# 18281818221/kalle-audio

Hardware: AMD Instinct MI355X
Metric: audio-seconds/sec (node) DiT train step, 10s@12.5Hz x1024 latents (higher is better)
Workload: dtype bf16; 1 GPU; DiT train step (fwd+bwd+allreduce+Adam), 24 blocks D=1536 h=24, 10 s @ 12.5 Hz x 1024 latents (T=125+1 prepend), S=130 x 768 cross-attn cond; DiT shape chosen by this build (reference defines none); global_batch=256, per_gpu_batch=256, parallelism=dp1, objective=v, io_channels=1024, global_cond_type=prepend

## Files before the change

### kalle_audio_amd/csrc/attention.hip

```cpp
#include "common.h"
#include "../../include/kalle_hip.h"

namespace {

template <int DH>
struct Hd {
    static_assert(DH == 32 || DH == 64 || DH == 128, "head dim 32, 64 or 128");
    static constexpr int STRIDE = 2 * DH + 32;
    static constexpr int TILE = 128 * STRIDE;
    static constexpr float SCALE = DH == 32 ? 0.17677669529663687f : DH == 64 ? 0.125f : 0.08838834764831845f;
    static constexpr float SCALE_LOG2E = SCALE * 1.4426950408889634f;
    static constexpr int PAIRS = DH / 16;
    static constexpr int PAIRS_LOG2 = DH == 32 ? 1 : DH == 64 ? 2 : 3;
    static constexpr int NP = DH == 128 ? 2 : 1;
};
constexpr int AT_STRIDE = Hd<64>::STRIDE;
constexpr int AT_TILE = Hd<64>::TILE;
constexpr float SM_SCALE = Hd<64>::SCALE;
constexpr float NEG_BIG = -1.0e30f;
constexpr float SM_SCALE_LOG2E = Hd<64>::SCALE_LOG2E;
constexpr float LOG2E = 1.4426950408889634f;
constexpr float M_INIT = -2.0e30f;

template <int NT, int DH = 64>
// ... 627 lines not shown
                            dp[t][ot] = __builtin_amdgcn_mfma_f32_16x16x32_bf16(x2, y2[ot][s], dp[t][ot], 0, 0, 0);
                        }
                    }
                    mfma_results_ready();
                    const f32x2 c2 = f32x2{SM_SCALE_LOG2E, SM_SCALE_LOG2E}, sc2 = f32x2{SM_SCALE, SM_SCALE};
                    const int ow = o0 + wave * (16 * OT);
                    const bool diag = p.causal && (KV ? (ow + 16 * OT - 1 > s0 + rb + coff) : (s0 + rb + 15 > ow + coff));
#pragma unroll
                    for (int ot = 0; ot < OT; ++ot) {
                        f32x2 la, lb, da, db;
                        if constexpr (KV) { la = lo2(ra); lb = hi2(ra); da = lo2(rbv); db = hi2(rbv); }
                        else { la = lb = f32x2{ca[ot], ca[ot]}; da = db = f32x2{cb[ot], cb[ot]}; }
                        const f32x2 ea = pk_fma(lo2(sa[t][ot]), c2, la), eb = pk_fma(hi2(sa[t][ot]), c2, lb);
                        f32x4 pv = f32x4{__builtin_amdgcn_exp2f(ea[0]), __builtin_amdgcn_exp2f(ea[1]),
                                         __builtin_amdgcn_exp2f(eb[0]), __builtin_amdgcn_exp2f(eb[1])};
                        if (diag) {
                            const int oi = ow + 16 * ot + li;
#pragma unroll
                            for (int r = 0; r < 4; ++r) {
                                const int si = s0 + rb + 4 * g + r;
                                if (KV ? (oi > si + coff) : (si > oi + coff)) pv[r] = 0.f;
                            }
                        }
                        const f32x2 ta = pk_fma(lo2(dp[t][ot]), sc2, da), tb = pk_fma(hi2(dp[t][ot]), sc2, db);
                        sa[t][ot] = pv;
                        dp[t][ot] = pv * f32x4{ta[0], ta[1], tb[0], tb[1]};
                    }
                }
                bf16x8 pb[OT], dsb[OT];
#pragma unroll
                for (int ot = 0; ot < OT; ++ot) {
                    pb[ot] = pack_pair(sa[0][ot], sa[1][ot]);
                    dsb[ot] = pack_pair(dp[0][ot], dp[1][ot]);
                }
#pragma unroll
                for (int dt = 0; dt < DT; ++dt) {
                    const bf16x8 a1 = trfrag<DH>(R1, 32 * pr, 32 * pr + 16, 16 * dt, lane);
#pragma unroll
                    for (int ot = 0; ot < OT; ++ot)
                        g2[dt][ot] = __builtin_amdgcn_mfma_f32_16x16x32_bf16(a1, dsb[ot], g2[dt][ot], 0, 0, 0);
                    if constexpr (KV) {
                        const bf16x8 a2 = trfrag<DH>(R2, 32 * pr, 32 * pr + 16, 16 * dt, lane);
#pragma unroll
                        for (int ot = 0; ot < OT; ++ot)
                            g1[dt][ot] = __builtin_amdgcn_mfma_f32_16x16x32_bf16(a2, pb[ot], g1[dt][ot], 0, 0, 0);
                    }
                }
            }
        }
    }

    const int nown = KV ? p.Nk : p.Nq;
#pragma unroll
    for (int ot = 0; ot < OT; ++ot) {
        const int oi = o0 + wave * (16 * OT) + 16 * ot + li;
        if (oi >= nown) continue;
        if (p.rot) {
            const int hts = p.rot >> 5;
#pragma unroll
            for (int ht = 0; ht < (DH == 32 ? 1 : 2); ++ht) {
                if (ht >= hts) break;
                const int64_t pos = oi + (KV ? 0 : p.qpos);
                const f32x4 c4 = *reinterpret_cast<const f32x4*>(p.cosT + pos * (p.rot >> 1) + 16 * ht + 4 * g);
                const f32x4 s4 = *reinterpret_cast<const f32x4*>(p.sinT + pos * (p.rot >> 1) + 16 * ht + 4 * g);
                f32x4& lo = hts == 1 ? g2[0][ot] : g2[ht][ot];
                f32x4& hi = hts == 1 ? g2[1][ot] : g2[DH == 32 ? 1 : ht + 2][ot];
#pragma unroll
                for (int r = 0; r < 4; ++r) {
                    const float a = lo[r], bb = hi[r];
                    lo[r] = a * c4[r] + bb * s4[r];
                    hi[r] = bb * c4[r] - a * s4[r];
                }
            }
        }
        if constexpr (KV) {
            bf16_t* dkp = p.dk + ((int64_t)b * p.Nk + oi) * p.ldk + p.k_off + hk * DH + 4 * g;
            bf16_t* dvp = p.dv + ((int64_t)b * p.Nk + oi) * p.ldv + p.v_off + hk * DH + 4 * g;
#pragma unroll
            for (int dt = 0; dt < DT; ++dt) {
                i32x2 w;
                w[0] = (int)pack_bf16x2(g2[dt][ot][0], g2[dt][ot][1]);
                w[1] = (int)pack_bf16x2(g2[dt][ot][2], g2[dt][ot][3]);
                *reinterpret_cast<i32x2*>(dkp + 16 * dt) = w;
                w[0] = (int)pack_bf16x2(g1[dt][ot][0], g1[dt][ot][1]);
                w[1] = (int)pack_bf16x2(g1[dt][ot][2], g1[dt][ot][3]);
                *reinterpret_cast<i32x2*>(dvp + 16 * dt) = w;
            }
        } else {
            bf16_t* dqp = p.dq + ((int64_t)b * p.Nq + oi) * p.ldq + p.q_off + hown * DH + 4 * g;
#pragma unroll
            for (int dt = 0; dt < DT; ++dt) {
                i32x2 w;
                w[0] = (int)pack_bf16x2(g2[dt][ot][0], g2[dt][ot][1]);
                w[1] = (int)pack_bf16x2(g2[dt][ot][2], g2[dt][ot][3]);
                *reinterpret_cast<i32x2*>(dqp + 16 * dt) = w;
            }
        }
    }
}

__device__ __forceinline__ float& row_stat(char* tile, int row, int slot) {
    return *reinterpret_cast<float*>(tile + row * AT_STRIDE + 128 + 4 * slot);
}

__global__ __launch_bounds__(512, 4) __attribute__((amdgpu_waves_per_eu(4, 4))) void attn_bwd_fused_kernel(AttnParams p) {
    constexpr int NT = 512;
    extern __shared__ __attribute__((aligned(16))) char smem[];
    char* RQ = smem;
    char* RD = smem + AT_TILE;
    char* RK = smem + 2 * AT_TILE;
    char* RV = smem + 3 * AT_TILE;
    const int tid = threadIdx.x, lane = tid & 63, wave = tid >> 6;
    const int g = lane >> 4, li = lane & 15;
    const int b = blockIdx.z, h = blockIdx.y;
    const int N = p.Nq, Nk = p.Nk;
    const bf16_t* qb = p.q + (int64_t)b * N * p.ldq + p.q_off + h * 64;
    const bf16_t* kb = p.k + (int64_t)b * Nk * p.ldk + p.k_off + h * 64;
    const bf16_t* vb = p.v + (int64_t)b * Nk * p.ldv + p.v_off + h * 64;
    const bf16_t* dob = p.dout + (int64_t)b * N * p.ldo + h * 64;
    attn_stamp(p, tid, 0);

    {
        TileRegs<NT> tq, td, tk, tv;
        tile_load<NT>(tq, qb, p.ldq, 0, N, p.rot, tid);
        tile_load<NT>(td, dob, p.ldo, 0, N, 0, tid);
        tile_load<NT>(tk, kb, p.ldk, 0, Nk, p.rot, tid);
        tile_load<NT>(tv, vb, p.ldv, 0, Nk, 0, tid);
        const RopeSet<> rq = rope_load(p.cosT, p.sinT, 0, N, p.rot, tid, p.qpos);
        const RopeSet<> rk = rope_load(p.cosT, p.sinT, 0, Nk, p.rot, tid);
        const int drow = tid >> 2, dq4 = tid & 3;
        i32x4 o0v = i32x4{0, 0, 0, 0}, o1v = i32x4{0, 0, 0, 0};
        if (drow < N) {
            const bf16_t* op = p.out + ((int64_t)b * N + drow) * p.ldo + h * 64 + 16 * dq4;
            o0v = *reinterpret_cast<const i32x4*>(op);
            o1v = *reinterpret_cast<const i32x4*>(op + 8);
        }
        float lse_pre = 0.f;
        bool key_ok = drow < Nk;
        if (dq4 == 0 && drow < N) lse_pre = p.lse[((int64_t)b * p.H + h) * N + drow];
        if (dq4 == 1 && key_ok && p.mask) key_ok = p.mask[(int64_t)b * Nk + drow] != 0;
        tile_store<NT>(RQ, tq, 0, N, p.cosT, p.sinT, p.rot, tid, p.qpos, p.rot != 0, rq);
        tile_store<NT>(RD, td, 0, N, nullptr, nullptr, 0, tid);
        tile_store<NT>(RK, tk, 0, Nk, p.cosT, p.sinT, p.rot, tid, 0, p.rot != 0, rk);
        tile_store<NT>(RV, tv, 0, Nk, nullptr, nullptr, 0, tid);
        __syncthreads();
        attn_stamp(p, tid, 1);
        const i32x4 d0v = *reinterpret_cast<const i32x4*>(RD + drow * AT_STRIDE + 32 * dq4);
        const i32x4 d1v = *reinterpret_cast<const i32x4*>(RD + drow * AT_STRIDE + 32 * dq4 + 16);
        float dl = 0.f;
#pragma unroll
        for (int e = 0; e < 4; ++e) {
            dl += bf16lo((uint32_t)o0v[e]) * bf16lo((uint32_t)d0v[e]) + bf16hi((uint32_t)o0v[e]) * bf16hi((uint32_t)d0v[e]);
            dl += bf16lo((uint32_t)o1v[e]) * bf16lo((uint32_t)d1v[e]) + bf16hi((uint32_t)o1v[e]) * bf16hi((uint32_t)d1v[e]);
        }
        dl += __shfl_xor(dl, 1, 64);
        dl += __shfl_xor(dl, 2, 64);
        if (dq4 == 0) {
            const bool ok = drow < N;
            row_stat(RQ, drow, 0) = ok ? -lse_pre * LOG2E : -INFINITY;
            row_stat(RQ, drow, 1) = ok ? -dl * SM_SCALE : 0.f;
            if (ok) p.delta[((int64_t)b * p.H + h) * N + drow] = dl;
        } else if (dq4 == 1) {
            row_stat(RK, drow, 0) = key_ok ? 0.f : -INFINITY;
        }
        __syncthreads();
    }
    attn_stamp(p, tid, 2);
    const f32x2 c2 = f32x2{SM_SCALE_LOG2E, SM_SCALE_LOG2E}, sc2 = f32x2{SM_SCALE, SM_SCALE};
    const int orow = wave * 16;

    if (orow < Nk) {
        bf16x8 y1[2], y2[2];
#pragma unroll
        for (int s = 0; s < 2; ++s) { y1[s] = rowfrag(RK, orow, s, lane); y2[s] = rowfrag(RV, orow, s, lane); }
        const float ca = row_stat(RK, orow + li, 0);
        f32x4 g1[4], g2[4];
#pragma unroll
        for (int dt = 0; dt < 4; ++dt) { g1[dt] = f32x4{0.f, 0.f, 0.f, 0.f}; g2[dt] = f32x4{0.f, 0.f, 0.f, 0.f}; }
#pragma unroll
        for (int pr = 0; pr < 4; ++pr) {
            if (32 * pr >= N) break;
            f32x4 sa[2], dp[2];
#pragma unroll
            for (int t = 0; t < 2; ++t) {
                const int rb = 32 * pr + 16 * t;
                sa[t] = f32x4{ca, ca, ca, ca};
                dp[t] = f32x4{0.f, 0.f, 0.f, 0.f};
#pragma unroll
                for (int s = 0; s < 2; ++s) {
                    sa[t] = __builtin_amdgcn_mfma_f32_16x16x32_bf16(rowfrag(RQ, rb, s, lane), y1[s], sa[t], 0, 0, 0);
                    dp[t] = __builtin_amdgcn_mfma_f32_16x16x32_bf16(rowfrag(RD, rb, s, lane), y2[s], dp[t], 0, 0, 0);
                }
                f32x4 ra, rbv;
#pragma unroll
                for (int r = 0; r < 4; ++r) { ra[r] = row_stat(RQ, rb + 4 * g + r, 0); rbv[r] = row_stat(RQ, rb + 4 * g + r, 1); }
                mfma_results_ready();
                const f32x2 ea = pk_fma(lo2(sa[t]), c2, lo2(ra)), eb = pk_fma(hi2(sa[t]), c2, hi2(ra));
                const f32x4 pv = f32x4{__builtin_amdgcn_exp2f(ea[0]), __builtin_amdgcn_exp2f(ea[1]),
                                       __builtin_amdgcn_exp2f(eb[0]), __builtin_amdgcn_exp2f(eb[1])};
                const f32x2 ta = pk_fma(lo2(dp[t]), sc2, lo2(rbv)), tb = pk_fma(hi2(dp[t]), sc2, hi2(rbv));
                sa[t] = pv;
                dp[t] = pv * f32x4{ta[0], ta[1], tb[0], tb[1]};
            }
            const bf16x8 pb = pack_pair(sa[0], sa[1]), dsb = pack_pair(dp[0], dp[1]);
#pragma unroll
            for (int dt = 0; dt < 4; ++dt) {
                g2[dt] = __builtin_amdgcn_mfma_f32_16x16x32_bf16(trfrag(RQ, 32 * pr, 32 * pr + 16, 16 * dt, lane), dsb, g2[dt], 0, 0, 0);
                g1[dt] = __builtin_amdgcn_mfma_f32_16x16x32_bf16(trfrag(RD, 32 * pr, 32 * pr + 16, 16 * dt, lane), pb, g1[dt], 0, 0, 0);
            }
        }
        attn_stamp(p, tid, 3);
        const int oi = orow + li;
        if (oi < Nk) {
            if (p.rot) {
                const int hts = p.rot >> 5;
#pragma unroll
                for (int ht = 0; ht < 2; ++ht) {
                    if (ht >= hts) break;
                    const f32x4 c4 = *reinterpret_cast<const f32x4*>(p.cosT + (int64_t)oi * (p.rot >> 1) + 16 * ht + 4 * g);
                    const f32x4 s4 = *reinterpret_cast<const f32x4*>(p.sinT + (int64_t)oi * (p.rot >> 1) + 16 * ht + 4 * g);
                    f32x4& lo = hts == 1 ? g2[0] : g2[ht];
                    f32x4& hi = hts == 1 ? g2[1] : g2[ht + 2];
#pragma unroll
                    for (int r = 0; r < 4; ++r) {
                        const float a = lo[r], bb = hi[r];
                        lo[r] = a * c4[r] + bb * s4[r];
                        hi[r] = bb * c4[r] - a * s4[r];
                    }
                }
            }
            store_row64(p.dk + ((int64_t)b * Nk + oi) * p.ldk + p.k_off + h * 64, g2[0], g2[1], g2[2], g2[3], g);
            store_row64(p.dv + ((int64_t)b * Nk + oi) * p.ldv + p.v_off + h * 64, g1[0], g1[1], g1[2], g1[3], g);
        }
    }

    attn_stamp(p, tid, 4);
    if (orow < N) {
        bf16x8 y1[2], y2[2];
#pragma unroll
        for (int s = 0; s < 2; ++s) { y1[s] = rowfrag(RQ, orow, s, lane); y2[s] = rowfrag(RD, orow, s, lane); }
        const float ca = row_stat(RQ, orow + li, 0), cb = row_stat(RQ, orow + li, 1);
        f32x4 g2[4];
#pragma unroll
        for (int dt = 0; dt < 4; ++dt) g2[dt] = f32x4{0.f, 0.f, 0.f, 0.f};
#pragma unroll
        for (int pr = 0; pr < 4; ++pr) {
            if (32 * pr >= Nk) break;
            f32x4 sa[2], dp[2];
#pragma unroll
            for (int t = 0; t < 2; ++t) {
                const int rb = 32 * pr + 16 * t;
#pragma unroll
                for (int r = 0; r < 4; ++r) sa[t][r] = row_stat(RK, rb + 4 * g + r, 0);
                dp[t] = f32x4{0.f, 0.f, 0.f, 0.f};
#pragma unroll
                for (int s = 0; s < 2; ++s) {
                    sa[t] = __builtin_amdgcn_mfma_f32_16x16x32_bf16(rowfrag(RK, rb, s, lane), y1[s], sa[t], 0, 0, 0);
                    dp[t] = __builtin_amdgcn_mfma_f32_16x16x32_bf16(rowfrag(RV, rb, s, lane), y2[s], dp[t], 0, 0, 0);
                }
                mfma_results_ready();
                const f32x2 la = f32x2{ca, ca}, da = f32x2{cb, cb};
                const f32x2 ea = pk_fma(lo2(sa[t]), c2, la), eb = pk_fma(hi2(sa[t]), c2, la);
                const f32x4 pv = f32x4{__builtin_amdgcn_exp2f(ea[0]), __builtin_amdgcn_exp2f(ea[1]),
                                       __builtin_amdgcn_exp2f(eb[0]), __builtin_amdgcn_exp2f(eb[1])};
                const f32x2 ta = pk_fma(lo2(dp[t]), sc2, da), tb = pk_fma(hi2(dp[t]), sc2, da);
                dp[t] = pv * f32x4{ta[0], ta[1], tb[0], tb[1]};
            }
            const bf16x8 dsb = pack_pair(dp[0], dp[1]);
#pragma unroll
            for (int dt = 0; dt < 4; ++dt)
                g2[dt] = __builtin_amdgcn_mfma_f32_16x16x32_bf16(trfrag(RK, 32 * pr, 32 * pr + 16, 16 * dt, lane), dsb, g2[dt], 0, 0, 0);
        }
        const int oi = orow + li;
        if (oi < N) {
            if (p.rot) {
                const int hts = p.rot >> 5;
#pragma unroll
                for (int ht = 0; ht < 2; ++ht) {
                    if (ht >= hts) break;
                    const int64_t pos = oi + p.qpos;
                    const f32x4 c4 = *reinterpret_cast<const f32x4*>(p.cosT + pos * (p.rot >> 1) + 16 * ht + 4 * g);
                    const f32x4 s4 = *reinterpret_cast<const f32x4*>(p.sinT + pos * (p.rot >> 1) + 16 * ht + 4 * g);
                    f32x4& lo = hts == 1 ? g2[0] : g2[ht];
                    f32x4& hi = hts == 1 ? g2[1] : g2[ht + 2];
#pragma unroll
                    for (int r = 0; r < 4; ++r) {
                        const float a = lo[r], bb = hi[r];
                        lo[r] = a * c4[r] + bb * s4[r];
                        hi[r] = bb * c4[r] - a * s4[r];
                    }
                }
            }
            attn_stamp(p, tid, 5);
            store_row64(p.dq + ((int64_t)b * N + oi) * p.ldq + p.q_off + h * 64, g2[0], g2[1], g2[2], g2[3], g);
        }
    }
    if (p.stamps) {
        attn_stamp(p, tid, 6);
        asm volatile("s_waitcnt vmcnt(0)" ::: "memory");
        attn_stamp(p, tid, 7);
    }
}

__global__ __launch_bounds__(512, 4) void attn_bwd_fused_gqa_kernel(AttnParams p) {
    constexpr int NT = 512;
    extern __shared__ __attribute__((aligned(16))) char smem[];
    char* RQ = smem;
    char* RD = smem + AT_TILE;
    char* RK = smem + 2 * AT_TILE;
    char* RV = smem + 3 * AT_TILE;
    const int tid = threadIdx.x, lane = tid & 63, wave = tid >> 6;
    const int g = lane >> 4, li = lane & 15;
    const int b = blockIdx.z, hk = blockIdx.y;
    const int group = p.H / p.Hkv;
    const int N = p.Nq, Nk = p.Nk;
    const int nmain = min(Nk, 128), tail = Nk - nmain;
    const int trow0 = 128 - tail;
    const bf16_t* kb = p.k + (int64_t)b * Nk * p.ldk + p.k_off + hk * 64;
    const bf16_t* vb = p.v + (int64_t)b * Nk * p.ldv + p.v_off + hk * 64;
    const f32x2 c2 = f32x2{SM_SCALE_LOG2E, SM_SCALE_LOG2E}, sc2 = f32x2{SM_SCALE, SM_SCALE};
    const int orow = wave * 16;
    const int drow = tid >> 2, dq4 = tid & 3;

    auto stage_head = [&](int h, bool with_kv, bool write_delta) {
        const bf16_t* qb = p.q + (int64_t)b * N * p.ldq + p.q_off + h * 64;
        const bf16_t* dob = p.dout + (int64_t)b * N * p.ldo + h * 64;
        TileRegs<NT> tq, td, tk, tv;
        tile_load<NT>(tq, qb, p.ldq, 0, N, 0, tid);
        tile_load<NT>(td, dob, p.ldo, 0, N, 0, tid);
        if (with_kv) {
            tile_load<NT>(tk, kb, p.ldk, 0, nmain, 0, tid);
            tile_load<NT>(tv, vb, p.ldv, 0, nmain, 0, tid);
        }
        i32x4 o0v = i32x4{0, 0, 0, 0}, o1v = i32x4{0, 0, 0, 0};
        if (drow < N) {
            const bf16_t* op = p.out + ((int64_t)b * N + drow) * p.ldo + h * 64 + 16 * dq4;
            o0v = *reinterpret_cast<const i32x4*>(op);
            o1v = *reinterpret_cast<const i32x4*>(op + 8);
        }
        i32x4 tkv = i32x4{0, 0, 0, 0}, tvv = i32x4{0, 0, 0, 0};
        const int tj = tid >> 3, tc = tid & 7;
        if (tj < tail) {
            tkv = *reinterpret_cast<const i32x4*>(kb + (int64_t)(128 + tj) * p.ldk + 8 * tc);
            tvv = *reinterpret_cast<const i32x4*>(vb + (int64_t)(128 + tj) * p.ldv + 8 * tc);
        }
        float lse_pre = 0.f;
        bool stat_ok = dq4 == 1 ? drow >= trow0 : drow < nmain;
        if (dq4 == 0 && drow < N) lse_pre = p.lse[((int64_t)b * p.H + h) * N + drow];
        if (dq4 == 1 && stat_ok && p.mask) stat_ok = p.mask[(int64_t)b * Nk + 128 + (drow - trow0)] != 0;
        if (dq4 == 2 && with_kv && stat_ok && p.mask) stat_ok = p.mask[(int64_t)b * Nk + drow] != 0;
        tile_store<NT>(RQ, tq, 0, N, nullptr, nullptr, 0, tid);
        tile_store<NT>(RD, td, 0, N, nullptr, nullptr, 0, tid);
        if (with_kv) {
            tile_store<NT>(RK, tk, 0, nmain, nullptr, nullptr, 0, tid);
            tile_store<NT>(RV, tv, 0, nmain, nullptr, nullptr, 0, tid);
        }
        __syncthreads();
        if (tj < tail) {
            *reinterpret_cast<i32x4*>(RQ + (trow0 + tj) * AT_STRIDE + 16 * tc) = tkv;
            *reinterpret_cast<i32x4*>(RD + (trow0 + tj) * AT_STRIDE + 16 * tc) = tvv;
        }
        const i32x4 d0v = *reinterpret_cast<const i32x4*>(RD + drow * AT_STRIDE + 32 * dq4);
        const i32x4 d1v = *reinterpret_cast<const i32x4*>(RD + drow * AT_STRIDE + 32 * dq4 + 16);
        float dl = 0.f;
#pragma unroll
        for (int e = 0; e < 4; ++e) {
            dl += bf16lo((uint32_t)o0v[e]) * bf16lo((uint32_t)d0v[e]) + bf16hi((uint32_t)o0v[e]) * bf16hi((uint32_t)d0v[e]);
            dl += bf16lo((uint32_t)o1v[e]) * bf16lo((uint32_t)d1v[e]) + bf16hi((uint32_t)o1v[e]) * bf16hi((uint32_t)d1v[e]);
        }
        dl += __shfl_xor(dl, 1, 64);
        dl += __shfl_xor(dl, 2, 64);
        if (dq4 == 0) {
            const bool ok = drow < N;
            row_stat(RQ, drow, 0) = ok ? -lse_pre * LOG2E : -INFINITY;
            row_stat(RQ, drow, 1) = ok ? -dl * SM_SCALE : 0.f;
            if (ok && write_delta) p.delta[((int64_t)b * p.H + h) * N + drow] = dl;
        } else if (dq4 == 1) {
            row_stat(RQ, drow, 2) = stat_ok ? 0.f : -INFINITY;
        } else if (dq4 == 2 && with_kv) {
            row_stat(RK, drow, 0) = stat_ok ? 0.f : -INFINITY;
        }
        __syncthreads();
    };

    auto keys_own = [&](const bf16x8 (&y1)[2], const bf16x8 (&y2)[2], float ca, f32x4 (&gv)[4], f32x4 (&gk)[4]) {
#pragma unroll
        for (int pr = 0; pr < 4; ++pr) {
            if (32 * pr >= N) break;
            f32x4 sa[2], dp[2];
#pragma unroll
            for (int t = 0; t < 2; ++t) {
                const int rb = 32 * pr + 16 * t;
                sa[t] = f32x4{ca, ca, ca, ca};
                dp[t] = f32x4{0.f, 0.f, 0.f, 0.f};
#pragma unroll
                for (int s = 0; s < 2; ++s) {
                    sa[t] = __builtin_amdgcn_mfma_f32_16x16x32_bf16(rowfrag(RQ, rb, s, lane), y1[s], sa[t], 0, 0, 0);
                    dp[t] = __builtin_amdgcn_mfma_f32_16x16x32_bf16(rowfrag(RD, rb, s, lane), y2[s], dp[t], 0, 0, 0);
                }
                f32x4 ra, rbv;
#pragma unroll
                for (int r = 0; r < 4; ++r) { ra[r] = row_stat(RQ, rb + 4 * g + r, 0); rbv[r] = row_stat(RQ, rb + 4 * g + r, 1); }
                mfma_results_ready();
                const f32x2 ea = pk_fma(lo2(sa[t]), c2, lo2(ra)), eb = pk_fma(hi2(sa[t]), c2, hi2(ra));
                f32x4 pv = f32x4{__builtin_amdgcn_exp2f(ea[0]), __builtin_amdgcn_exp2f(ea[1]),
                                 __builtin_amdgcn_exp2f(eb[0]), __builtin_amdgcn_exp2f(eb[1])};
                const f32x2 ta = pk_fma(lo2(dp[t]), sc2, lo2(rbv)), tb = pk_fma(hi2(dp[t]), sc2, hi2(rbv));
                f32x4 ds = pv * f32x4{ta[0], ta[1], tb[0], tb[1]};
#pragma unroll
                for (int r = 0; r < 4; ++r) {
                    if (rb + 4 * g + r >= N) { pv[r] = 0.f; ds[r] = 0.f; }
                }
                sa[t] = pv;
                dp[t] = ds;
            }
            const bf16x8 pb = pack_pair(sa[0], sa[1]), dsb = pack_pair(dp[0], dp[1]);
#pragma unroll
            for (int dt = 0; dt < 4; ++dt) {
                gk[dt] = __builtin_amdgcn_mfma_f32_16x16x32_bf16(trfrag(RQ, 32 * pr, 32 * pr + 16, 16 * dt, lane), dsb, gk[dt], 0, 0, 0);
                gv[dt] = __builtin_amdgcn_mfma_f32_16x16x32_bf16(trfrag(RD, 32 * pr, 32 * pr + 16, 16 * dt, lane), pb, gv[dt], 0, 0, 0);
            }
        }
    };

    {
        stage_head(hk * group, true, true);
        f32x4 g1[4], g2[4];
#pragma unroll
        for (int dt = 0; dt < 4; ++dt) { g1[dt] = f32x4{0.f, 0.f, 0.f, 0.f}; g2[dt] = f32x4{0.f, 0.f, 0.f, 0.f}; }
        for (int hh = 0; hh < group; ++hh) {
            if (hh > 0) {
                __syncthreads();
                stage_head(hk * group + hh, false, true);
            }
            if (orow < nmain) {
                bf16x8 y1[2], y2[2];
#pragma unroll
                for (int s = 0; s < 2; ++s) { y1[s] = rowfrag(RK, orow, s, lane); y2[s] = rowfrag(RV, orow, s, lane); }
                keys_own(y1, y2, row_stat(RK, orow + li, 0), g1, g2);
            }
        }
        const int oi = orow + li;
        if (oi < nmain) {
            store_row64(p.dk + ((int64_t)b * Nk + oi) * p.ldk + p.k_off + hk * 64, g2[0], g2[1], g2[2], g2[3], g);
            store_row64(p.dv + ((int64_t)b * Nk + oi) * p.ldv + p.v_off + hk * 64, g1[0], g1[1], g1[2], g1[3], g);
        }
    }

    for (int hh = group - 1; hh >= 0; --hh) {
        const int h = hk * group + hh;
        if (hh != group - 1) {
            __syncthreads();
            stage_head(h, false, false);
        }
        if (orow < N) {
            bf16x8 y1[2], y2[2];
#pragma unroll
            for (int s = 0; s < 2; ++s) { y1[s] = rowfrag(RQ, orow, s, lane); y2[s] = rowfrag(RD, orow, s, lane); }
            const float ca = row_stat(RQ, orow + li, 0), cb = row_stat(RQ, orow + li, 1);
            f32x4 gq[4];
#pragma unroll
            for (int dt = 0; dt < 4; ++dt) gq[dt] = f32x4{0.f, 0.f, 0.f, 0.f};
            auto stream_keys = [&](const char* SK, const char* SV, int base, auto ext_c) {
                constexpr bool EXT = decltype(ext_c)::value;
                f32x4 dp[2];
#pragma unroll
                for (int t = 0; t < (EXT ? 1 : 2); ++t) {
                    dp[t] = f32x4{0.f, 0.f, 0.f, 0.f};
                    const int rb = base + 16 * t;
                    f32x4 sa;
#pragma unroll
                    for (int r = 0; r < 4; ++r) sa[r] = EXT ? row_stat(RQ, rb + 4 * g + r, 2) : row_stat(RK, rb + 4 * g + r, 0);
#pragma unroll
                    for (int s = 0; s < 2; ++s) {
                        sa = __builtin_amdgcn_mfma_f32_16x16x32_bf16(rowfrag(SK, rb, s, lane), y1[s], sa, 0, 0, 0);
                        dp[t] = __builtin_amdgcn_mfma_f32_16x16x32_bf16(rowfrag(SV, rb, s, lane), y2[s], dp[t], 0, 0, 0);
                    }
                    mfma_results_ready();
                    const f32x2 la = f32x2{ca, ca}, da = f32x2{cb, cb};
                    const f32x2 ea = pk_fma(lo2(sa), c2, la), eb = pk_fma(hi2(sa), c2, la);
                    const f32x4 pv = f32x4{__builtin_amdgcn_exp2f(ea[0]), __builtin_amdgcn_exp2f(ea[1]),
                                           __builtin_amdgcn_exp2f(eb[0]), __builtin_amdgcn_exp2f(eb[1])};
                    const f32x2 ta = pk_fma(lo2(dp[t]), sc2, da), tb = pk_fma(hi2(dp[t]), sc2, da);
                    f32x4 ds = pv * f32x4{ta[0], ta[1], tb[0], tb[1]};
                    if constexpr (EXT) {
#pragma unroll
                        for (int r = 0; r < 4; ++r)
                            if (rb + 4 * g + r < trow0) ds[r] = 0.f;
                    }
                    dp[t] = ds;
                }
                if constexpr (EXT) dp[1] = f32x4{0.f, 0.f, 0.f, 0.f};
                const bf16x8 dsb = pack_pair(dp[0], dp[1]);
                const int rb_ = EXT ? base : base + 16;
#pragma unroll
                for (int dt = 0; dt < 4; ++dt)
                    gq[dt] = __builtin_amdgcn_mfma_f32_16x16x32_bf16(trfrag(SK, base, rb_, 16 * dt, lane), dsb, gq[dt], 0, 0, 0);
            };
#pragma unroll 1
            for (int pr = 0; pr < 4; ++pr) {
                if (32 * pr >= nmain) break;
                stream_keys(RK, RV, 32 * pr, std::false_type{});
            }
            if (tail > 0) stream_keys(RQ, RD, 112, std::true_type{});
            const int oi = orow + li;
            if (oi < N) {
                store_row64(p.dq + ((int64_t)b * N + oi) * p.ldq + p.q_off + h * 64, gq[0], gq[1], gq[2], gq[3], g);
            }
        }
        if (tail > 0 && wave == 7) {
            f32x4 gt1[4], gt2[4];
#pragma unroll
            for (int dt = 0; dt < 4; ++dt) {
                if (hh == group - 1) { gt1[dt] = f32x4{0.f, 0.f, 0.f, 0.f}; gt2[dt] = f32x4{0.f, 0.f, 0.f, 0.f}; }
                else {
                    gt1[dt] = *reinterpret_cast<const f32x4*>(RD + (2 * lane + (dt >> 1)) * AT_STRIDE + 128 + 16 * (dt & 1));
                    gt2[dt] = *reinterpret_cast<const f32x4*>(RV + (2 * lane + (dt >> 1)) * AT_STRIDE + 128 + 16 * (dt & 1));
                }
            }
            bf16x8 y1[2], y2[2];
#pragma unroll
            for (int s = 0; s < 2; ++s) { y1[s] = rowfrag(RQ, 112, s, lane); y2[s] = rowfrag(RD, 112, s, lane); }
            keys_own(y1, y2, row_stat(RQ, 112 + li, 2), gt1, gt2);
            if (hh > 0) {
#pragma unroll
                for (int dt = 0; dt < 4; ++dt) {
                    *reinterpret_cast<f32x4*>(RD + (2 * lane + (dt >> 1)) * AT_STRIDE + 128 + 16 * (dt & 1)) = gt1[dt];
                    *reinterpret_cast<f32x4*>(RV + (2 * lane + (dt >> 1)) * AT_STRIDE + 128 + 16 * (dt & 1)) = gt2[dt];
                }
            } else {
                const int row = 112 + li;
                if (row >= trow0) {
                    const int key = 128 + (row - trow0);
                    store_row64(p.dk + ((int64_t)b * Nk + key) * p.ldk + p.k_off + hk * 64, gt2[0], gt2[1], gt2[2], gt2[3], g);
                    store_row64(p.dv + ((int64_t)b * Nk + key) * p.ldv + p.v_off + hk * 64, gt1[0], gt1[1], gt1[2], gt1[3], g);
                }
            }
        }
    }
}

bool check_common(const void* q, int64_t ldq, int q_off, const void* k, int64_t ldk, int k_off, const void* v,
                  int64_t ldv, int v_off, int64_t ldo, int rot, int B, int H, int Hkv, int Nq, int Nk) {
    if (!q || !k || !v || B <= 0 || H <= 0 || Hkv <= 0 || Nq <= 0 || Nk <= 0) return false;
    if (H % Hkv) return false;
    if ((ldq & 7) || (ldk & 7) || (ldv & 7) || (ldo & 7) || (q_off & 7) || (k_off & 7) || (v_off & 7)) return false;
    if (rot != 0 && rot != 32 && rot != 64) return false;
    if (H > 65535 || B > 65535) return false;
    return true;
}

template <int ROT>
__global__ __launch_bounds__(256) void attn_decode_kernel(AttnParams p) {
    extern __shared__ __attribute__((aligned(16))) char smem[];
    float* sc = reinterpret_cast<float*>(smem);
    __shared__ float qs[64];
    __shared__ float red[8];
    __shared__ float osum[4][64];
    constexpr int HALF = ROT / 2;
    const int tid = threadIdx.x, lane = tid & 63, wave = tid >> 6;
    const int h = blockIdx.x, b = blockIdx.y;
    const int hk = h / (p.H / p.Hkv);
    const bf16_t* qsrc = p.q + (int64_t)b * p.ldq + p.q_off + h * 64;
    const bf16_t* ksrc = p.k + (int64_t)b * p.Nk * p.ldk + p.k_off + hk * 64;
    const bf16_t* vsrc = p.v + (int64_t)b * p.Nk * p.ldv + p.v_off + hk * 64;
    auto rnd = [](float x) { return bf16_to_f32(f32_to_bf16(x)); };

    if (tid < 64) {
        float x = bf16_to_f32(qsrc[tid]);
        if constexpr (ROT > 0) {
            if (tid < ROT) {
                const bool lo = tid < HALF;
                const float partner = bf16_to_f32(qsrc[lo ? tid + HALF : tid - HALF]);
                const int i = lo ? tid : tid - HALF;
                const float c = p.cosT[(int64_t)p.qpos * HALF + i], sn = p.sinT[(int64_t)p.qpos * HALF + i];
                x = rnd(x * c + (lo ? -partner : partner) * sn);
            }
        }
        qs[tid] = x;
    }
    __syncthreads();

    float mx = NEG_BIG;
    for (int j = tid; j < p.Nk; j += 256) {
        const bf16_t* kp = ksrc + (int64_t)j * p.ldk;
        float kf[64];
#pragma unroll
        for (int c = 0; c < 8; ++c) {
            const i32x4 w = reinterpret_cast<const i32x4*>(kp)[c];
#pragma unroll
            for (int e = 0; e < 4; ++e) {
                kf[8 * c + 2 * e] = bf16lo((uint32_t)w[e]);
                kf[8 * c + 2 * e + 1] = bf16hi((uint32_t)w[e]);
            }
        }
        if constexpr (ROT > 0) {
            const float* cp = p.cosT + (int64_t)j * HALF;
            const float* sp = p.sinT + (int64_t)j * HALF;
#pragma unroll
            for (int i4 = 0; i4 < HALF / 4; ++i4) {
                const f32x4 c = reinterpret_cast<const f32x4*>(cp)[i4], sn = reinterpret_cast<const f32x4*>(sp)[i4];
#pragma unroll
                for (int e = 0; e < 4; ++e) {
                    const int i = 4 * i4 + e;
                    const float a = kf[i], bb = kf[i + HALF];
                    kf[i] = rnd(a * c[e] - bb * sn[e]);
                    kf[i + HALF] = rnd(bb * c[e] + a * sn[e]);
                }
            }
        }
        float a0 = 0.f, a1 = 0.f;
#pragma unroll
        for (int d = 0; d < 64; d += 2) { a0 += kf[d] * qs[d]; a1 += kf[d + 1] * qs[d + 1]; }
        float sv = (a0 + a1) * SM_SCALE;
        if (p.mask && !p.mask[(int64_t)b * p.Nk + j]) sv = NEG_BIG;
        sc[j] = sv;
        mx = fmaxf(mx, sv);
    }
#pragma unroll
    for (int o = 32; o > 0; o >>= 1) mx = fmaxf(mx, __shfl_xor(mx, o, 64));
    if (lane == 0) red[wave] = mx;
    __syncthreads();
    const float m = fmaxf(fmaxf(red[0], red[1]), fmaxf(red[2], red[3]));
    float ls = 0.f;
    for (int j = tid; j < p.Nk; j += 256) {
        const float pv = __expf(sc[j] - m);
        ls += pv;
        sc[j] = rnd(pv);
    }
#pragma unroll
    for (int o = 32; o > 0; o >>= 1) ls += __shfl_xor(ls, o, 64);
    if (lane == 0) red[4 + wave] = ls;
    __syncthreads();
    const float l = red[4] + red[5] + red[6] + red[7];

    const int kg = tid >> 3, d8 = tid & 7;
    float acc[8];
#pragma unroll
    for (int e = 0; e < 8; ++e) acc[e] = 0.f;
#pragma unroll 4
    for (int j = kg; j < p.Nk; j += 32) {
        const i32x4 w = *reinterpret_cast<const i32x4*>(vsrc + (int64_t)j * p.ldv + 8 * d8);
        const float pj = sc[j];
#pragma unroll
        for (int e = 0; e < 4; ++e) {
            acc[2 * e] += pj * bf16lo((uint32_t)w[e]);
            acc[2 * e + 1] += pj * bf16hi((uint32_t)w[e]);
        }
    }
#pragma unroll
    for (int e = 0; e < 8; ++e) {
        acc[e] += __shfl_xor(acc[e], 8, 64);
        acc[e] += __shfl_xor(acc[e], 16, 64);
        acc[e] += __shfl_xor(acc[e], 32, 64);
    }
    if (lane < 8) {
#pragma unroll
        for (int e = 0; e < 8; ++e) osum[wave][8 * lane + e] = acc[e];
    }
    __syncthreads();
    if (tid < 64) {
        const float o = (osum[0][tid] + osum[1][tid] + osum[2][tid] + osum[3][tid]) / l;
        p.out[(int64_t)b * p.ldo + h * 64 + tid] = f32_to_bf16(o);
        if (tid == 0 && p.lse) p.lse[(int64_t)b * p.H + h] = m + __logf(l);
    }
}

}

static unsigned long long* g_attn_stamps = nullptr;
extern "C" int kalle_attn_debug_stamps(void* buf) { g_attn_stamps = static_cast<unsigned long long*>(buf); return KALLE_OK; }

template <int DH>
static int attention_fwd_dh(const AttnParams& p, hipStream_t st) {
    constexpr int lds = 3 * Hd<DH>::TILE + 160 * 4 + 2 * 32 * Hd<DH>::STRIDE;
    static std::atomic<uint64_t> lds_ok{0};
    kalle_allow_lds(reinterpret_cast<const void*>(attn_fwd_kernel<1, DH>), lds, lds_ok);
    KALLE_LAUNCH((attn_fwd_kernel<1, DH>), dim3((p.Nq + 127) / 128, p.H, p.B), dim3(512), lds, st, p);
    return kalle_check_launch();
}
template <int DH>
static int attention_bwd_dh(const AttnParams& p, hipStream_t st) {
    constexpr int lds = 2 * Hd<DH>::TILE + 256 * 4;
    static std::atomic<uint64_t> lds_ok_kv{0}, lds_ok_q{0};
    kalle_allow_lds(reinterpret_cast<const void*>(attn_bwd_kernel<true, 1, DH>), lds, lds_ok_kv);
    kalle_allow_lds(reinterpret_cast<const void*>(attn_bwd_kernel<false, 1, DH>), lds, lds_ok_q);
    KALLE_LAUNCH((attn_bwd_kernel<false, 1, DH>), dim3((p.Nq + 127) / 128, p.H, p.B), dim3(512), lds, st, p);
    KALLE_LAUNCH((attn_bwd_kernel<true, 1, DH>), dim3((p.Nk + 127) / 128, p.Hkv, p.B), dim3(512), lds, st, p);
    return kalle_check_launch();
}
static bool check_head_dim(int head_dim, int rot) {
    return (head_dim == 32 || head_dim == 64 || head_dim == 128) && rot <= head_dim;
}

extern "C" int kalle_attention_fwd_hd(const void* q, int64_t ldq, int q_off, const void* k, int64_t ldk, int k_off,
                                      const void* v, int64_t ldv, int v_off, void* out, int64_t ldo, float* lse,
                                      const float* rope_cos, const float* rope_sin, int rot, const uint8_t* key_mask,
                                      int causal, int B, int H, int Hkv, int Nq, int Nk, int head_dim, void* stream) {
    if (!out || !check_common(q, ldq, q_off, k, ldk, k_off, v, ldv, v_off, ldo, rot, B, H, Hkv, Nq, Nk) ||
        !check_head_dim(head_dim, rot))
        return KALLE_ERR_ARG;
    if (rot && (!rope_cos || !rope_sin)) return KALLE_ERR_ARG;
    AttnParams p{};
    p.q = static_cast<const bf16_t*>(q); p.ldq = ldq; p.q_off = q_off;
    p.k = static_cast<const bf16_t*>(k); p.ldk = ldk; p.k_off = k_off;
    p.v = static_cast<const bf16_t*>(v); p.ldv = ldv; p.v_off = v_off;
    p.out = static_cast<bf16_t*>(out); p.ldo = ldo; p.lse = lse;
    p.cosT = rope_cos; p.sinT = rope_sin; p.rot = rot; p.mask = key_mask;
    p.B = B; p.H = H; p.Hkv = Hkv; p.Nq = Nq; p.Nk = Nk; p.causal = causal;
    p.stamps = g_attn_stamps;
    if (causal && Nk < Nq) return KALLE_ERR_ARG;
    p.qpos = causal ? Nk - Nq : 0;
    if (head_dim == 32) return attention_fwd_dh<32>(p, static_cast<hipStream_t>(stream));
    if (head_dim == 128) return attention_fwd_dh<128>(p, static_cast<hipStream_t>(stream));
    if (Nq == 1 && Nk <= 15360) {
        const dim3 grid(H, B), block(256);
        hipStream_t st = static_cast<hipStream_t>(stream);
        if (rot == 64) KALLE_LAUNCH(attn_decode_kernel<64>, grid, block, (size_t)Nk * 4, st, p);
        else if (rot == 32) KALLE_LAUNCH(attn_decode_kernel<32>, grid, block, (size_t)Nk * 4, st, p);
        else KALLE_LAUNCH(attn_decode_kernel<0>, grid, block, (size_t)Nk * 4, st, p);
        return kalle_check_launch();
    }
    constexpr int lds = 3 * AT_TILE + 160 * 4 + 2 * 32 * AT_STRIDE;
    static std::atomic<uint64_t> lds_ok{0};
    kalle_allow_lds(reinterpret_cast<const void*>(attn_fwd_kernel<1>), lds, lds_ok);
    dim3 grid((Nq + 127) / 128, H, B), block(512);
    KALLE_LAUNCH(attn_fwd_kernel<1>, grid, block, lds, static_cast<hipStream_t>(stream), p);
    return kalle_check_launch();
}

extern "C" int kalle_attention_bwd_hd(const void* q, int64_t ldq, int q_off, const void* k, int64_t ldk, int k_off,
                                      const void* v, int64_t ldv, int v_off, const void* out, const void* dout,
                                      int64_t ldo, const float* lse, float* delta, void* dq, void* dk, void* dv,
                                      const float* rope_cos, const float* rope_sin, int rot, const uint8_t* key_mask,
                                      int causal, int B, int H, int Hkv, int Nq, int Nk, int head_dim, void* stream) {
    if (!out || !dout || !lse || !delta || !dq || !dk || !dv ||
        !check_common(q, ldq, q_off, k, ldk, k_off, v, ldv, v_off, ldo, rot, B, H, Hkv, Nq, Nk) ||
        !check_head_dim(head_dim, rot))
        return KALLE_ERR_ARG;
    if (rot && (!rope_cos || !rope_sin)) return KALLE_ERR_ARG;
    hipStream_t st = static_cast<hipStream_t>(stream);
    AttnParams p{};
    p.q = static_cast<const bf16_t*>(q); p.ldq = ldq; p.q_off = q_off;
    p.k = static_cast<const bf16_t*>(k); p.ldk = ldk; p.k_off = k_off;
    p.v = static_cast<const bf16_t*>(v); p.ldv = ldv; p.v_off = v_off;
    p.out = static_cast<bf16_t*>(const_cast<void*>(out)); p.ldo = ldo; p.lse = const_cast<float*>(lse);
    p.cosT = rope_cos; p.sinT = rope_sin; p.rot = rot; p.mask = key_mask;
    p.B = B; p.H = H; p.Hkv = Hkv; p.Nq = Nq; p.Nk = Nk; p.causal = causal;
    if (causal && Nk < Nq) return KALLE_ERR_ARG;
    p.qpos = causal ? Nk - Nq : 0;
    p.dout = static_cast<const bf16_t*>(dout); p.delta = delta;
    p.dq = static_cast<bf16_t*>(dq); p.dk = static_cast<bf16_t*>(dk); p.dv = static_cast<bf16_t*>(dv);
    p.stamps = g_attn_stamps;
    if (head_dim == 32) return attention_bwd_dh<32>(p, st);
    if (head_dim == 128) return attention_bwd_dh<128>(p, st);

    if (!causal && Nq <= 128 && Nk <= 128 && H == Hkv) {
        constexpr int flds = 4 * AT_TILE;
        static std::atomic<uint64_t> lds_ok_f{0};
        kalle_allow_lds(reinterpret_cast<const void*>(attn_bwd_fused_kernel), flds, lds_ok_f);
        KALLE_LAUNCH(attn_bwd_fused_kernel, dim3(1, H, B), dim3(512), flds, st, p);
        return kalle_check_launch();
    }
    const int tail = Nk > 128 ? Nk - 128 : 0;
    if (!causal && rot == 0 && Nq <= 128 && tail <= 16 && tail <= 128 - Nq) {
        constexpr int flds = 4 * AT_TILE;
        static std::atomic<uint64_t> lds_ok_g{0};
        kalle_allow_lds(reinterpret_cast<const void*>(attn_bwd_fused_gqa_kernel), flds, lds_ok_g);
        KALLE_LAUNCH(attn_bwd_fused_gqa_kernel, dim3(1, Hkv, B), dim3(512), flds, st, p);
        return kalle_check_launch();
    }
    constexpr int lds = 2 * AT_TILE + 256 * 4;
    static std::atomic<uint64_t> lds_ok_kv{0}, lds_ok_q{0};
    kalle_allow_lds(reinterpret_cast<const void*>(attn_bwd_kernel<true, 1>), lds, lds_ok_kv);
    kalle_allow_lds(reinterpret_cast<const void*>(attn_bwd_kernel<false, 1>), lds, lds_ok_q);
    KALLE_LAUNCH((attn_bwd_kernel<false, 1>), dim3((Nq + 127) / 128, H, B), dim3(512), lds, st, p);
    KALLE_LAUNCH((attn_bwd_kernel<true, 1>), dim3((Nk + 127) / 128, Hkv, B), dim3(512), lds, st, p);
    return kalle_check_launch();
}

extern "C" int kalle_attention_fwd(const void* q, int64_t ldq, int q_off, const void* k, int64_t ldk, int k_off,
                                   const void* v, int64_t ldv, int v_off, void* out, int64_t ldo, float* lse,
                                   const float* rope_cos, const float* rope_sin, int rot, const uint8_t* key_mask,
                                   int causal, int B, int H, int Hkv, int Nq, int Nk, void* stream) {
    return kalle_attention_fwd_hd(q, ldq, q_off, k, ldk, k_off, v, ldv, v_off, out, ldo, lse, rope_cos, rope_sin, rot, key_mask,
                                  causal, B, H, Hkv, Nq, Nk, 64, stream);
}
extern "C" int kalle_attention_bwd(const void* q, int64_t ldq, int q_off, const void* k, int64_t ldk, int k_off,
                                   const void* v, int64_t ldv, int v_off, const void* out, const void* dout,
                                   int64_t ldo, const float* lse, float* delta, void* dq, void* dk, void* dv,
                                   const float* rope_cos, const float* rope_sin, int rot, const uint8_t* key_mask,
                                   int causal, int B, int H, int Hkv, int Nq, int Nk, void* stream) {
    return kalle_attention_bwd_hd(q, ldq, q_off, k, ldk, k_off, v, ldv, v_off, out, dout, ldo, lse, delta, dq, dk, dv, rope_cos,
                                  rope_sin, rot, key_mask, causal, B, H, Hkv, Nq, Nk, 64, stream);
}
```

Measured before the change: 11640 audio-seconds/sec.

## Prefetch next head's Q/dO/out into registers during current head's GQA backward compute

```diff
diff --git a/kalle_audio_amd/csrc/attention.hip b/kalle_audio_amd/csrc/attention.hip
--- a/kalle_audio_amd/csrc/attention.hip
+++ b/kalle_audio_amd/csrc/attention.hip
@@ -953,6 +953,26 @@
     }
 }
 
+__device__ __forceinline__ float delta_chain(const i32x4& oa, const i32x4& ob, const i32x4& da, const i32x4& db) {
+    auto lo = [](int w) { return bf16lo((uint32_t)w); };
+    auto hi = [](int w) { return bf16hi((uint32_t)w); };
+    float dl = hi(oa[0]) * hi(da[0]);
+    dl = __builtin_fmaf(lo(oa[0]), lo(da[0]), dl);
+#pragma unroll
+    for (int e = 1; e < 4; ++e) {
+        dl = __builtin_fmaf(hi(oa[e]), hi(da[e]), dl);
+        dl = __builtin_fmaf(lo(oa[e]), lo(da[e]), dl);
+    }
+    dl = __builtin_fmaf(lo(ob[0]), lo(db[0]), dl);
+    dl = __builtin_fmaf(hi(ob[0]), hi(db[0]), dl);
+#pragma unroll
+    for (int e = 1; e < 4; ++e) {
+        dl = __builtin_fmaf(hi(ob[e]), hi(db[e]), dl);
+        dl = __builtin_fmaf(lo(ob[e]), lo(db[e]), dl);
+    }
+    return dl;
+}
+
 __global__ __launch_bounds__(512, 4) void attn_bwd_fused_gqa_kernel(AttnParams p) {
     constexpr int NT = 512;
     extern __shared__ __attribute__((aligned(16))) char smem[];
@@ -973,64 +993,69 @@
     const int orow = wave * 16;
     const int drow = tid >> 2, dq4 = tid & 3;
 
-    auto stage_head = [&](int h, bool with_kv, bool write_delta) {
-        const bf16_t* qb = p.q + (int64_t)b * N * p.ldq + p.q_off + h * 64;
-        const bf16_t* dob = p.dout + (int64_t)b * N * p.ldo + h * 64;
-        TileRegs<NT> tq, td, tk, tv;
-        tile_load<NT>(tq, qb, p.ldq, 0, N, 0, tid);
-        tile_load<NT>(td, dob, p.ldo, 0, N, 0, tid);
-        if (with_kv) {
-            tile_load<NT>(tk, kb, p.ldk, 0, nmain, 0, tid);
-            tile_load<NT>(tv, vb, p.ldv, 0, nmain, 0, tid);
-        }
-        i32x4 o0v = i32x4{0, 0, 0, 0}, o1v = i32x4{0, 0, 0, 0};
-        if (drow < N) {
-            const bf16_t* op = p.out + ((int64_t)b * N + drow) * p.ldo + h * 64 + 16 * dq4;
-            o0v = *reinterpret_cast<const i32x4*>(op);
-            o1v = *reinterpret_cast<const i32x4*>(op + 8);
-        }
-        i32x4 tkv = i32x4{0, 0, 0, 0}, tvv = i32x4{0, 0, 0, 0};
-        const int tj = tid >> 3, tc = tid & 7;
-        if (tj < tail) {
-            tkv = *reinterpret_cast<const i32x4*>(kb + (int64_t)(128 + tj) * p.ldk + 8 * tc);
-            tvv = *reinterpret_cast<const i32x4*>(vb + (int64_t)(128 + tj) * p.ldv + 8 * tc);
-        }
-        float lse_pre = 0.f;
+    struct HeadRegs { i32x4 q0, q1, d0, d1, o0, o1; float lse, dl; };
+    auto head_issue = [&](HeadRegs& r, int h, bool with_tail, auto from_delta_c) {
+        constexpr bool FROM_DELTA = decltype(from_delta_c)::value;
+        int t = tid;
+        asm volatile("" : "+v"(t));
+        const int row = t >> 2, j = t & 3;
+        r.q0 = r.q1 = r.d0 = r.d1 = r.o0 = r.o1 = i32x4{0, 0, 0, 0};
+        r.lse = 0.f; r.dl = 0.f;
+        if (row < N) {
+            const bf16_t* qp = p.q + ((int64_t)b * N + row) * p.ldq + p.q_off + h * 64 + 16 * j;
+            const bf16_t* dp = p.dout + ((int64_t)b * N + row) * p.ldo + h * 64 + 16 * j;
+            r.q0 = *reinterpret_cast<const i32x4*>(qp); r.q1 = *reinterpret_cast<const i32x4*>(qp + 8);
+            r.d0 = *reinterpret_cast<const i32x4*>(dp); r.d1 = *reinterpret_cast<const i32x4*>(dp + 8);
+            if constexpr (!FROM_DELTA) {
+                const bf16_t* op = p.out + ((int64_t)b * N + row) * p.ldo + h * 64 + 16 * j;
+                r.o0 = *reinterpret_cast<const i32x4*>(op); r.o1 = *reinterpret_cast<const i32x4*>(op + 8);
+            }
+            if (j == 0) {
+                r.lse = p.lse[((int64_t)b * p.H + h) * N + row];
+                if constexpr (FROM_DELTA) r.dl = p.delta[((int64_t)b * p.H + h) * N + row];
+            }
+        } else if (with_tail && row >= trow0) {
+            const bf16_t* kp = kb + (int64_t)(128 + row - trow0) * p.ldk + 16 * j;
+            const bf16_t* vp = vb + (int64_t)(128 + row - trow0) * p.ldv + 16 * j;
+            r.q0 = *reinterpret_cast<const i32x4*>(kp); r.q1 = *reinterpret_cast<const i32x4*>(kp + 8);
+            r.d0 = *reinterpret_cast<const i32x4*>(vp); r.d1 = *reinterpret_cast<const i32x4*>(vp + 8);
+        }
+    };
+    auto head_commit = [&](const HeadRegs& r, int h, bool all_rows, auto from_delta_c) {
+        constexpr bool FROM_DELTA = decltype(from_delta_c)::value;
+        if (all_rows || drow < N) {
+            *reinterpret_cast<i32x4*>(RQ + drow * AT_STRIDE + 32 * dq4) = r.q0;
+            *reinterpret_cast<i32x4*>(RQ + drow * AT_STRIDE + 32 * dq4 + 16) = r.q1;
+            *reinterpret_cast<i32x4*>(RD + drow * AT_STRIDE + 32 * dq4) = r.d0;
+            *reinterpret_cast<i32x4*>(RD + drow * AT_STRIDE + 32 * dq4 + 16) = r.d1;
+        }
+        float dl = r.dl;
+        if constexpr (!FROM_DELTA) {
+            dl = delta_chain(r.o0, r.o1, r.d0, r.d1);
+            dl += __shfl_xor(dl, 1, 64);
+            dl += __shfl_xor(dl, 2, 64);
+        }
+        if (dq4 == 0 && (all_rows || drow < N)) {
+            const bool ok = drow < N;
+            row_stat(RQ, drow, 0) = ok ? -r.lse * LOG2E : -INFINITY;
+            row_stat(RQ, drow, 1) = ok ? -dl * SM_SCALE : 0.f;
+            if (ok && !FROM_DELTA) p.delta[((int64_t)b * p.H + h) * N + drow] = dl;
+        }
+    };
+    auto stage_first = [&](int h) {
+        HeadRegs r;
+        TileRegs<NT> tk, tv;
+        head_issue(r, h, true, std::false_type{});
+        tile_load<NT>(tk, kb, p.ldk, 0, nmain, 0, tid);
+        tile_load<NT>(tv, vb, p.ldv, 0, nmain, 0, tid);
         bool stat_ok = dq4 == 1 ? drow >= trow0 : drow < nmain;
-        if (dq4 == 0 && drow < N) lse_pre = p.lse[((int64_t)b * p.H + h) * N + drow];
         if (dq4 == 1 && stat_ok && p.mask) stat_ok = p.mask[(int64_t)b * Nk + 128 + (drow - trow0)] != 0;
-        if (dq4 == 2 && with_kv && stat_ok && p.mask) stat_ok = p.mask[(int64_t)b * Nk + drow] != 0;
-        tile_store<NT>(RQ, tq, 0, N, nullptr, nullptr, 0, tid);
-        tile_store<NT>(RD, td, 0, N, nullptr, nullptr, 0, tid);
-        if (with_kv) {
-            tile_store<NT>(RK, tk, 0, nmain, nullptr, nullptr, 0, tid);
-            tile_store<NT>(RV, tv, 0, nmain, nullptr, nullptr, 0, tid);
-        }
-        __syncthreads();
-        if (tj < tail) {
-            *reinterpret_cast<i32x4*>(RQ + (trow0 + tj) * AT_STRIDE + 16 * tc) = tkv;
-            *reinterpret_cast<i32x4*>(RD + (trow0 + tj) * AT_STRIDE + 16 * tc) = tvv;
-        }
-        const i32x4 d0v = *reinterpret_cast<const i32x4*>(RD + drow * AT_STRIDE + 32 * dq4);
-        const i32x4 d1v = *reinterpret_cast<const i32x4*>(RD + drow * AT_STRIDE + 32 * dq4 + 16);
-        float dl = 0.f;
-#pragma unroll
-        for (int e = 0; e < 4; ++e) {
-            dl += bf16lo((uint32_t)o0v[e]) * bf16lo((uint32_t)d0v[e]) + bf16hi((uint32_t)o0v[e]) * bf16hi((uint32_t)d0v[e]);
-            dl += bf16lo((uint32_t)o1v[e]) * bf16lo((uint32_t)d1v[e]) + bf16hi((uint32_t)o1v[e]) * bf16hi((uint32_t)d1v[e]);
-        }
-        dl += __shfl_xor(dl, 1, 64);
-        dl += __shfl_xor(dl, 2, 64);
-        if (dq4 == 0) {
-            const bool ok = drow < N;
-            row_stat(RQ, drow, 0) = ok ? -lse_pre * LOG2E : -INFINITY;
-            row_stat(RQ, drow, 1) = ok ? -dl * SM_SCALE : 0.f;
-            if (ok && write_delta) p.delta[((int64_t)b * p.H + h) * N + drow] = dl;
-        } else if (dq4 == 1) {
-            row_stat(RQ, drow, 2) = stat_ok ? 0.f : -INFINITY;
-        } else if (dq4 == 2 && with_kv) {
-            row_stat(RK, drow, 0) = stat_ok ? 0.f : -INFINITY;
-        }
+        if (dq4 == 2 && stat_ok && p.mask) stat_ok = p.mask[(int64_t)b * Nk + drow] != 0;
+        head_commit(r, h, true, std::false_type{});
+        tile_store<NT>(RK, tk, 0, nmain, nullptr, nullptr, 0, tid);
+        tile_store<NT>(RV, tv, 0, nmain, nullptr, nullptr, 0, tid);
+        if (dq4 == 1) row_stat(RQ, drow, 2) = stat_ok ? 0.f : -INFINITY;
+        else if (dq4 == 2) row_stat(RK, drow, 0) = stat_ok ? 0.f : -INFINITY;
         __syncthreads();
     };
 
@@ -1075,20 +1100,24 @@
     };
 
     {
-        stage_head(hk * group, true, true);
+        stage_first(hk * group);
         f32x4 g1[4], g2[4];
 #pragma unroll
         for (int dt = 0; dt < 4; ++dt) { g1[dt] = f32x4{0.f, 0.f, 0.f, 0.f}; g2[dt] = f32x4{0.f, 0.f, 0.f, 0.f}; }
         for (int hh = 0; hh < group; ++hh) {
-            if (hh > 0) {
-                __syncthreads();
-                stage_head(hk * group + hh, false, true);
-            }
+            const bool more = hh + 1 < group;
+            HeadRegs nx;
+            if (more) head_issue(nx, hk * group + hh + 1, false, std::false_type{});
             if (orow < nmain) {
                 bf16x8 y1[2], y2[2];
 #pragma unroll
                 for (int s = 0; s < 2; ++s) { y1[s] = rowfrag(RK, orow, s, lane); y2[s] = rowfrag(RV, orow, s, lane); }
                 keys_own(y1, y2, row_stat(RK, orow + li, 0), g1, g2);
+            }
+            if (more) {
+                __syncthreads();
+                head_commit(nx, hk * group + hh + 1, false, std::false_type{});
+                __syncthreads();
             }
         }
         const int oi = orow + li;
@@ -1100,10 +1129,9 @@
 
     for (int hh = group - 1; hh >= 0; --hh) {
         const int h = hk * group + hh;
-        if (hh != group - 1) {
-            __syncthreads();
-            stage_head(h, false, false);
-        }
+        const bool more = hh > 0;
+        HeadRegs nx;
+        if (more) head_issue(nx, h - 1, false, std::true_type{});
         if (orow < N) {
             bf16x8 y1[2], y2[2];
 #pragma unroll
@@ -1187,6 +1215,11 @@
                     store_row64(p.dv + ((int64_t)b * Nk + key) * p.ldv + p.v_off + hk * 64, gt1[0], gt1[1], gt1[2], gt1[3], g);
                 }
             }
+        }
+        if (more) {
+            __syncthreads();
+            head_commit(nx, h - 1, false, std::true_type{});
+            __syncthreads();
         }
     }
 }
```

Result: no change. 11650 audio-seconds/sec (median of 2 runs) (+0.1%).
